# BraveGroup/DCD

Hardware: AMD Instinct MI355X
Metric: images/sec DGDE train step (bs=8, 384x1280) (higher is better)
Workload: dtype f32; 1 GPU; DGDE train bs=8 fp32 on 1xMI355X, synthetic KITTI 384x1280 + random kpts_ann (DGDE.yaml, DLA-34+DCNv2, 6 objects/image); global_batch=8, per_gpu_batch=8, input=384x1280, parallelism=dp1, dcn_precision=f32, step_launch=eager, sync_bn=False

## Files before the change

### dcd_amd/_lib.py

```python
import ctypes
import os

_HERE = os.path.dirname(os.path.abspath(__file__))
LIB_PATH = os.path.join(_HERE, "libdcd_hip.so")
_LIB = None

c_void_p, c_int, c_float, c_size_t, c_int64, c_double = (ctypes.c_void_p, ctypes.c_int, ctypes.c_float,
                                                         ctypes.c_size_t, ctypes.c_int64, ctypes.c_double)


class LossRowsArgs(ctypes.Structure):
    _INTS = ("B", "M", "C", "K", "NP", "num_classes", "ch_box2d", "ch_offset", "ch_corner", "ch_corner_unc", "ch_dims",
             "ch_ori_cls", "ch_ori_off", "ch_depth", "ch_depth_unc", "ch_kpts2d", "ch_kpts3d", "trunc_log")
    _FLOATS = ("depth_lo", "depth_hi", "unc_lo", "unc_hi", "depth_weight")
    _POINTERS = ("pois", "reg_mask", "trunc_mask", "find_pcl", "ori_mask", "cls_ids", "centers", "pad_size", "bboxes",
                 "locations", "rotys", "offset_3D", "dimensions", "orientations", "keypoints", "kp_depth_mask", "kpts2d",
                 "kpts3d", "calib_P", "calib", "dim_mean", "kps_pred", "kps_tgt", "kps3d_pred", "kps3d_tgt", "rot", "P_rows",
                 "kmask", "pair_depth", "pair_mask", "cols", "corners_pred", "corners_tgt", "iou3d", "sums", "grad_sums",
                 "grad_pois", "grad_pair", "grad_kps", "grad_kps3d")
    _fields_ = ([(n, c_int) for n in _INTS] + [(n, c_float) for n in _FLOATS] + [("dim_weight", c_float * 3)]
                + [("down_ratio", c_float), ("kd_eps", c_float)] + [(n, c_void_p) for n in _POINTERS])

HEADS_MAX = 16

# ... 48 lines not shown
    "dcd_nms_hm": (c_int, [c_void_p, c_void_p, c_int, c_int, c_int, c_int, c_void_p]),
    "dcd_heatmap_topk": (c_int, [c_void_p, c_void_p] + [c_int] * 6 + [c_void_p] * 5 + [c_void_p, c_size_t]),
    "dcd_heatmap_topk_workspace_bytes": (c_size_t, [c_int] * 5),
    "dcd_poi_gather": (c_int, [c_void_p, c_void_p, c_void_p] + [c_int] * 5 + [c_void_p]),
    "dcd_poi_scatter_add": (c_int, [c_void_p, c_void_p, c_void_p] + [c_int] * 5 + [c_void_p]),
    "dcd_patch_scatter_add": (c_int, [c_void_p, c_void_p, c_void_p, c_int, c_int, c_int64, c_int, c_int, c_void_p]),
    "dcd_iou3d": (c_int, [c_void_p, c_void_p, c_void_p, c_int, c_void_p]),
    "dcd_conv3x3_workspace_bytes": (c_size_t, [c_int] * 5),
    "dcd_conv3x3": (c_int, [c_void_p] * 6 + [c_int] * 6 + [c_void_p, c_size_t]),
    "dcd_conv3x3_weights_bytes": (c_size_t, [c_int] * 3),
    "dcd_conv3x3_transform_weights": (c_int, [c_void_p, c_void_p, c_int, c_int, c_void_p, c_void_p]),
    "dcd_conv3x3_transform_weights_table": (c_int, [c_void_p, c_void_p, c_int]),
    "dcd_conv3x3_prepared": (c_int, [c_void_p] * 6 + [c_int] * 6 + [c_void_p, c_size_t]),
    "dcd_conv3x3_split_weights_bytes": (c_size_t, [c_int] * 3),
    "dcd_conv3x3_split_transform_weights": (c_int, [c_void_p, c_void_p, c_int, c_int, c_void_p, c_void_p]),
    "dcd_conv3x3_split_transform_weights_table": (c_int, [c_void_p, c_void_p, c_int]),
    "dcd_conv3x3_split_workspace_bytes": (c_size_t, [c_int] * 5),
    "dcd_conv3x3_split_prepared": (c_int, [c_void_p] * 6 + [c_int] * 7 + [c_void_p, c_size_t]),
    "dcd_conv1x1_bf16": (c_int, [c_void_p, c_void_p, c_int, c_int, c_int, c_void_p, c_void_p, c_void_p, c_int, c_int, c_int64]),
    "dcd_conv1x1_wrw_bf16_workspace_bytes": (c_size_t, [c_int, c_int, c_int, c_int64]),
    "dcd_conv1x1_wrw_bf16": (c_int, [c_void_p, c_void_p, c_void_p, c_void_p, c_int, c_int, c_int, c_int, c_int64, c_void_p, c_size_t]),
    "dcd_conv3x3_s2_f32": (c_int, [c_void_p, c_void_p, c_void_p, c_void_p, c_int, c_int, c_int, c_int, c_int]),
    "dcd_conv3x3_s2_f32_backward_data": (c_int, [c_void_p, c_void_p, c_void_p, c_void_p, c_int, c_int, c_int, c_int, c_int]),
    "dcd_conv3x3_s2_f32_wrw_workspace_bytes": (c_size_t, [c_int, c_int, c_int, c_int, c_int]),
    "dcd_conv3x3_s2_f32_wrw": (c_int, [c_void_p, c_void_p, c_void_p, c_void_p, c_int, c_int, c_int, c_int, c_int, c_void_p, c_size_t]),
    "dcd_clip_adamw_workspace_bytes": (c_size_t, [c_int, c_void_p]),
    "dcd_clip_grad_norm_scalars": (c_int, [c_void_p, c_int, c_void_p, c_void_p, c_float, c_void_p, c_size_t, c_void_p]),
    "dcd_adamw_apply": (c_int, [c_void_p, c_int] + [c_void_p] * 7 + [c_double] * 4 + [c_void_p]),
    "dcd_conv1x1_f32": (c_int, [c_void_p, c_void_p, c_int, c_int, c_int, c_void_p, c_void_p, c_void_p, c_int, c_int, c_int64]),
    "dcd_conv1x1_wrw_f32_workspace_bytes": (c_size_t, [c_int, c_int, c_int, c_int64]),
    "dcd_conv1x1_wrw_f32": (c_int, [c_void_p, c_void_p, c_void_p, c_void_p, c_int, c_int, c_int, c_int, c_int64, c_void_p, c_size_t]),
    "dcd_conv3x3_bf16_weights_bytes": (c_size_t, [c_int] * 3),
    "dcd_conv3x3_bf16_transform_weights": (c_int, [c_void_p, c_void_p, c_int, c_int, c_void_p, c_void_p]),
    "dcd_conv3x3_bf16_transform_weights_table": (c_int, [c_void_p, c_void_p, c_int]),
    "dcd_conv3x3_bf16_workspace_bytes": (c_size_t, [c_int] * 5),
    "dcd_conv3x3_bf16_prepared": (c_int, [c_void_p] * 6 + [c_int] * 6 + [c_void_p, c_size_t]),
    "dcd_conv_stem_workspace_bytes": (c_size_t, [c_int] * 3),
    "dcd_conv_stem": (c_int, [c_void_p] * 4 + [c_int] * 7 + [c_void_p, c_size_t]),
    "dcd_conv_stem_wrw_workspace_bytes": (c_size_t, [c_int] * 3),
    "dcd_conv_stem_wrw": (c_int, [c_void_p] * 4 + [c_int] * 6 + [c_void_p, c_size_t]),
    "dcd_context_norm_forward": (c_int, [c_void_p] * 4 + [c_int, c_int, c_float]),
    "dcd_context_norm_backward": (c_int, [c_void_p] * 5 + [c_int, c_int]),
    "dcd_context_norm_relu_add_forward": (c_int, [c_void_p] * 4 + [c_int, c_int, c_float]),
    "dcd_gmw_refine": (c_int, [c_void_p] * 5 + [c_int, c_void_p, c_void_p, c_int, c_int, c_int] + [c_void_p] * 3),
    "dcd_gmw_pack_records": (c_int, [c_void_p] * 4 + [c_int, c_int, c_void_p, c_int, c_int, c_int] + [c_void_p] * 9),
    "dcd_sum_tensors": (c_int, [c_void_p, c_void_p, c_int, c_void_p, c_int64]),
    "dcd_conv3x3_wrw_workspace_bytes": (c_size_t, [c_int] * 5),
    "dcd_conv3x3_wrw": (c_int, [c_void_p] * 4 + [c_int] * 6 + [c_void_p, c_size_t]),
    "dcd_upsample_dw_forward": (c_int, [c_void_p] * 4 + [c_int] * 5),
    "dcd_upsample_dw_forward_add": (c_int, [c_void_p] * 5 + [c_int] * 5),
    "dcd_maxpool2x2_forward": (c_int, [c_void_p, c_void_p, c_void_p, c_int64, c_int, c_int]),
    "dcd_maxpool2x2_backward": (c_int, [c_void_p, c_void_p, c_void_p, c_void_p, c_int64, c_int, c_int]),
    "dcd_upsample_dw_backward": (c_int, [c_void_p] * 6 + [c_int] * 5),
    "dcd_bn_workspace_bytes": (c_size_t, [c_int]),
    "dcd_bn_stats": (c_int, [c_void_p, c_void_p, c_int, c_int, c_int64, c_void_p, c_void_p, c_size_t]),
    "dcd_channel_sums": (c_int, [c_void_p, c_void_p, c_int, c_int, c_int64, c_void_p, c_void_p, c_size_t]),
    "dcd_bn_train_apply": (c_int, [c_void_p] * 6 + [c_double] + [c_void_p] * 3 + [c_float, c_float, c_int] + [c_void_p] * 3
                           + [c_int, c_int, c_int64]),
    "dcd_bn_eval_apply": (c_int, [c_void_p] * 7 + [c_float, c_int, c_void_p, c_int, c_int, c_int64]),
    "dcd_bn_backward_stats": (c_int, [c_void_p] * 5 + [c_int, c_int, c_int64, c_void_p, c_void_p, c_size_t]),
    "dcd_trunk_row_sums": (c_int, [c_void_p, c_void_p, c_void_p, c_int, c_int, c_void_p]),
    "dcd_trunk_finalize_forward": (c_int, [c_void_p, c_void_p, c_void_p, c_void_p, c_double, c_double, c_int, c_void_p, c_void_p, c_void_p]),
    "dcd_trunk_finalize_backward": (c_int, [c_void_p, c_void_p, c_void_p, c_void_p, c_void_p, c_double, c_int, c_void_p, c_void_p, c_void_p]),
    "dcd_trunk_grad_wg": (c_int, [c_void_p, c_void_p, c_void_p, c_int, c_int, c_void_p]),
    "dcd_bn_backward_relu_from_x": (c_int, [c_void_p] * 10 + [c_int, c_int, c_int64, c_void_p, c_size_t]),
    "dcd_bn_backward_stats_params_relu_from_x": (c_int, [c_void_p] * 7 + [c_int, c_int, c_int64, c_void_p, c_void_p, c_void_p, c_void_p, c_size_t]),
    "dcd_bn_backward_apply_relu_from_x": (c_int, [c_void_p] * 8 + [c_double, c_void_p, c_int, c_int, c_int64]),
    "dcd_bn_backward_stats_params": (c_int, [c_void_p] * 6 + [c_int, c_int, c_int64, c_void_p, c_void_p, c_void_p, c_void_p, c_size_t]),
    "dcd_bn_backward_apply": (c_int, [c_void_p] * 8 + [c_double] + [c_void_p] * 4 + [c_int, c_int, c_int64]),
    "dcd_bn_at_forward": (c_int, [c_void_p] * 6 + [c_double] + [c_void_p] * 3 + [c_float, c_float, c_int] + [c_void_p] * 4
                          + [c_int, c_int, c_int64, c_int] + [c_void_p, c_size_t]),
    "dcd_bn_at_backward_sums": (c_int, [c_void_p] * 7 + [c_int, c_int, c_int] + [c_void_p, c_void_p]),
    "dcd_bn_train_forward": (c_int, [c_void_p] * 8 + [c_float, c_float, c_int] + [c_void_p] * 3 + [c_int, c_int, c_int64]
                             + [c_void_p, c_size_t]),
    "dcd_bn_backward": (c_int, [c_void_p] * 11 + [c_int, c_int, c_int64] + [c_void_p, c_size_t]),
# ... 82 lines not shown
```

### dcd_amd/csrc/conv.hip

```cpp
#include <hip/hip_runtime.h>
#include <stdint.h>
#include <stdlib.h>

#include "../../include/dcd_hip.h"
#include "tuning_env.h"
#include "lds_limit.h"
#include "bf16_split.h"

typedef float f32x16 __attribute__((ext_vector_type(16)));
typedef float f32x4 __attribute__((ext_vector_type(4)));
typedef float f32x2 __attribute__((ext_vector_type(2)));

namespace {

constexpr int WN_CH = 8;
constexpr int WN_NT = 512;

template <int TR, int TC, int NB>
struct WinoGeom {
    static constexpr int KS = 32 * NB;
    static constexpr int U = 16 * KS * WN_CH;
    static constexpr int NTILE = TR * TC;
    static constexpr int ROWS = 4 * TR + 2;
    static constexpr int Q = (2 * TC + 8) / 4;
// ... 1398 lines not shown

static bool s2_args_ok(int B, int Cin, int H, int W, int Cout)
{
    return B > 0 && Cin > 0 && Cout > 0 && H > 0 && W > 0 && (H & 1) == 0 && (W & 7) == 0 && (Cin & 15) == 0 &&
           (int64_t)Cin * H * W < (1ll << 29) && (int64_t)Cout * (H / 2) * (W / 2) < (1ll << 29);
}

int dcd_conv3x3_s2_f32(void *stream_, const float *input, const float *weight, float *output, int B, int Cin, int H, int W, int Cout)
{
    (void)hipGetLastError();
    if (!input || !weight || !output || !s2_args_ok(B, Cin, H, W, Cout)) return DCD_ERR_BAD_ARG;
    S2Args a;
    a.x = input; a.w = weight; a.y = output; a.B = B; a.C = Cin; a.H = H; a.W = W; a.K = Cout; a.Ho = H / 2; a.Wo = W / 2;
    const int zb = (Cout + 31) / 32;
    const bool small = (int64_t)((a.Ho * a.Wo + 511) / 512) * B * zb < (int64_t)device_cus();
    if (small) hipLaunchKernelGGL(s2_conv_f32<2>, dim3((unsigned)((a.Ho * a.Wo + 255) / 256), B, zb), dim3(S2_NT), 0, (hipStream_t)stream_, a);
    else hipLaunchKernelGGL(s2_conv_f32<4>, dim3((unsigned)((a.Ho * a.Wo + 511) / 512), B, zb), dim3(S2_NT), 0, (hipStream_t)stream_, a);
    return hipGetLastError() == hipSuccess ? DCD_OK : DCD_ERR_LAUNCH;
}

int dcd_conv3x3_s2_f32_backward_data(void *stream_, const float *grad_output, const float *weight, float *grad_input, int B, int Cin, int H,
                                     int W, int Cout)
{
    (void)hipGetLastError();
    if (!grad_output || !weight || !grad_input || !s2_args_ok(B, Cin, H, W, Cout) || (Cout & 15)) return DCD_ERR_BAD_ARG;
    S2Args a;
    a.x = grad_output; a.w = weight; a.y = grad_input; a.B = B; a.C = Cin; a.H = H; a.W = W; a.K = Cout; a.Ho = H / 2; a.Wo = W / 2;
    const int zb = (Cin + 31) / 32;
    const bool small = (int64_t)((a.Ho * a.Wo + 511) / 512) * B * 2 * zb < (int64_t)device_cus();
    if (small) hipLaunchKernelGGL(s2_dgrad_f32<2>, dim3((unsigned)((a.Ho * a.Wo + 255) / 256), B, 2 * zb), dim3(S2_NT), 0, (hipStream_t)stream_, a);
    else hipLaunchKernelGGL(s2_dgrad_f32<4>, dim3((unsigned)((a.Ho * a.Wo + 511) / 512), B, 2 * zb), dim3(S2_NT), 0, (hipStream_t)stream_, a);
    return hipGetLastError() == hipSuccess ? DCD_OK : DCD_ERR_LAUNCH;
}

static int s2_wrw_splits(int B, int Cin, int H, int W, int Cout)
{
    const int nblk = ((Cout + 31) / 32) * ((Cin + 31) / 32);
    const int64_t groups = (int64_t)B * (H / 2) * (W / 2) / 8;
    int64_t S = (8 * (int64_t)device_cus() + nblk - 1) / nblk;
    if (S > groups / 8) S = groups / 8;
    if (S < 1) S = 1;
    return (int)S;
}

size_t dcd_conv3x3_s2_f32_wrw_workspace_bytes(int B, int Cin, int H, int W, int Cout)
{
    if (!s2_args_ok(B, Cin, H, W, Cout)) return 0;
    return (size_t)s2_wrw_splits(B, Cin, H, W, Cout) * 9 * Cout * Cin * sizeof(float);
}

// ... 93 lines not shown
```

### dcd_amd/csrc/conv_s2_f32.inc

```

constexpr int S2_NT = 256;

struct S2Args {
    const float *x, *w;
    float *y;
    int B, C, H, W, K, Ho, Wo;
};

template <int NPX> struct S2WinT { float v[3][2 * NPX + 1]; };
typedef S2WinT<4> S2Win;

template <int NPX>
__device__ __forceinline__ void s2_gather(const __amdgpu_buffer_rsrc_t rs, const int (&off_l)[3], const int (&off_v)[3], int soff, S2WinT<NPX> &w)
{
#pragma unroll
    for (int a = 0; a < 3; ++a) {
        w.v[a][0] = __builtin_bit_cast(float, __builtin_amdgcn_raw_buffer_load_b32(rs, off_l[a], soff, 0));
        const f32x4 p = __builtin_bit_cast(f32x4, __builtin_amdgcn_raw_buffer_load_b128(rs, off_v[a], soff, 0));
        w.v[a][1] = p.x; w.v[a][2] = p.y; w.v[a][3] = p.z; w.v[a][4] = p.w;
        if constexpr (NPX == 4) {
            const f32x4 q = __builtin_bit_cast(f32x4, __builtin_amdgcn_raw_buffer_load_b128(rs, off_v[a] + 16, soff, 0));
            w.v[a][5] = q.x; w.v[a][6] = q.y; w.v[a][7] = q.z; w.v[a][8] = q.w;
        }
    }
}

template <int NPX>
__global__ __launch_bounds__(S2_NT, 2) void s2_conv_f32(S2Args a)
{
// ... 129 lines not shown
        }
        __syncthreads();
#pragma unroll
        for (int j = 0; j < 8; ++j) {
            const int kn = ck * 8 + j + DEP;
            if (kn < nk) gather(((kn >> 3) * 16 + (kn & 7)) * HWo * 4, win[(j + DEP) % NBUF]);
            const Win &w = win[j % NBUF];
#pragma unroll
            for (int ia = 0; ia < NR; ++ia) {
                const int ta = PY ? (ia == 0 ? 0 : 2) : 1, r = PY ? (ia == 0 ? 1 : 0) : 0;
#pragma unroll
                for (int tb = 0; tb < 3; ++tb) {
                    const int px = tb == 1 ? 0 : 1, dm = tb == 0 ? 1 : 0;
                    const float A = wl[((ta * 3 + tb) * 2 + (j >> 2)) * 64 + lane][j & 3];
#pragma unroll
                    for (int t = 0; t < NPX; ++t)
                        acc[px][t] = __builtin_amdgcn_mfma_f32_32x32x2f32(A, w.g[r][t + dm], acc[px][t], 0, 0, 0);
                }
            }
        }
    }
    if (!pv) return;
    float *o_b = a.y + (size_t)b * a.C * HW + (size_t)(2 * i + PY) * a.W + 2 * j0;
#pragma unroll
    for (int r = 0; r < 16; ++r) {
        const int c = z * 32 + (r & 3) + 8 * (r >> 2) + 4 * kg;
        if (c < a.C) {
            *reinterpret_cast<f32x4 *>(o_b + (size_t)c * HW) = f32x4{acc[0][0][r], acc[1][0][r], acc[0][1][r], acc[1][1][r]};
            if constexpr (NPX == 4)
                *reinterpret_cast<f32x4 *>(o_b + (size_t)c * HW + 4) = f32x4{acc[0][2][r], acc[1][2][r], acc[0][3][r], acc[1][3][r]};
        }
    }
}

template <int NPX>
__global__ __launch_bounds__(S2_NT, 2) void s2_dgrad_f32(S2Args a)
{
    __shared__ __attribute__((aligned(16))) f32x4 wl[9 * 2 * 64];
    if (blockIdx.z & 1) s2_dgrad_body<1, NPX>(a, wl, blockIdx.z >> 1);
    else s2_dgrad_body<0, NPX>(a, wl, blockIdx.z >> 1);
}

struct S2WrwArgs {
    const float *x, *gy;
    float *part;
    int B, C, H, W, K, Ho, Wo, S, ncb;
// ... 92 lines not shown
```

### dcd_amd/csrc/upsample.hip

```cpp
#include <hip/hip_runtime.h>
#include <stdlib.h>

#include <cstdint>
#include <stdint.h>

#include "../../include/dcd_hip.h"
#include "tuning_env.h"
#include "zero_fill.h"

namespace {

template <int F>
__global__ __launch_bounds__(256) void up_dw_fwd(const float *__restrict__ x, const float *__restrict__ w, float *__restrict__ y,
                                                 int C, int H, int W, const float *__restrict__ skip)
{
    constexpr int K = 2 * F, P = F / 2;
    __shared__ float ws[K * K];
    const int plane = blockIdx.y, c = plane % C;
    for (int i = threadIdx.x; i < K * K; i += 256) ws[i] = w[(size_t)c * K * K + i];
    __syncthreads();
    const int Ho = H * F, Wo = W * F;
    const float *xp = x + (size_t)plane * H * W;
    float *yp = y + (size_t)plane * Ho * Wo;
    const int o0 = (blockIdx.x * 256 + threadIdx.x) * 4;
// ... 169 lines not shown
    if (c > m || c != c) { m = c; k = 2; }
    if (d > m || d != d) { m = d; k = 3; }
    return k;
}

__global__ __launch_bounds__(256) void maxpool2_fwd(const float *__restrict__ x, float *__restrict__ y, int64_t planes, int H, int W)
{
    const int Ho = H / 2, Wq = W / 4;
    const int64_t n = planes * Ho * Wq;
    for (int64_t i = (int64_t)blockIdx.x * 256 + threadIdx.x; i < n; i += (int64_t)gridDim.x * 256) {
        const int q = (int)(i % Wq);
        const int64_t r = i / Wq;
        const int oy = (int)(r % Ho);
        const int64_t pl = r / Ho;
        const float *p = x + (pl * H + 2 * oy) * W + 4 * q;
        const float4 t = *reinterpret_cast<const float4 *>(p), b = *reinterpret_cast<const float4 *>(p + W);
        float m0, m1;
        argmax4(t.x, t.y, b.x, b.y, m0);
        argmax4(t.z, t.w, b.z, b.w, m1);
        *reinterpret_cast<float2 *>(y + (pl * Ho + oy) * (W / 2) + 2 * q) = make_float2(m0, m1);
    }
}

__global__ __launch_bounds__(256) void maxpool2_bwd(const float *__restrict__ x, const float *__restrict__ gy, float *__restrict__ gx,
                                                    int64_t planes, int H, int W)
{
    const int Ho = H / 2, Wq = W / 4;
    const int64_t n = planes * Ho * Wq;
    for (int64_t i = (int64_t)blockIdx.x * 256 + threadIdx.x; i < n; i += (int64_t)gridDim.x * 256) {
        const int q = (int)(i % Wq);
        const int64_t r = i / Wq;
        const int oy = (int)(r % Ho);
        const int64_t pl = r / Ho;
        const size_t o = (size_t)(pl * H + 2 * oy) * W + 4 * q;
        const float4 t = *reinterpret_cast<const float4 *>(x + o), b = *reinterpret_cast<const float4 *>(x + o + W);
        const float2 g = *reinterpret_cast<const float2 *>(gy + (pl * Ho + oy) * (W / 2) + 2 * q);
        float m;
        const int k0 = argmax4(t.x, t.y, b.x, b.y, m), k1 = argmax4(t.z, t.w, b.z, b.w, m);
        const float4 gt = make_float4(k0 == 0 ? g.x : 0.f, k0 == 1 ? g.x : 0.f, k1 == 0 ? g.y : 0.f, k1 == 1 ? g.y : 0.f);
        const float4 gb = make_float4(k0 == 2 ? g.x : 0.f, k0 == 3 ? g.x : 0.f, k1 == 2 ? g.y : 0.f, k1 == 3 ? g.y : 0.f);
        *reinterpret_cast<float4 *>(gx + o) = gt;
        *reinterpret_cast<float4 *>(gx + o + W) = gb;
    }
}

}

extern "C" {

int dcd_maxpool2x2_forward(void *stream_, const float *x, float *y, int64_t planes, int H, int W)
{
    (void)hipGetLastError();
    if (!x || !y || planes <= 0 || H < 2 || W < 4 || (H & 1) || (W & 3) || (((uintptr_t)x | (uintptr_t)y) & 15)) return DCD_ERR_BAD_ARG;
    const int64_t n = planes * (H / 2) * (W / 4);
    const unsigned grid = (unsigned)((n + 255) / 256 < 65535 * 4 ? (n + 255) / 256 : 65535 * 4);
    hipLaunchKernelGGL(maxpool2_fwd, dim3(grid), dim3(256), 0, (hipStream_t)stream_, x, y, planes, H, W);
    return hipGetLastError() == hipSuccess ? DCD_OK : DCD_ERR_LAUNCH;
}

int dcd_maxpool2x2_backward(void *stream_, const float *x, const float *grad_y, float *grad_x, int64_t planes, int H, int W)
{
    (void)hipGetLastError();
    if (!x || !grad_y || !grad_x || planes <= 0 || H < 2 || W < 4 || (H & 1) || (W & 3) ||
        (((uintptr_t)x | (uintptr_t)grad_y | (uintptr_t)grad_x) & 15))
        return DCD_ERR_BAD_ARG;
    const int64_t n = planes * (H / 2) * (W / 4);
    const unsigned grid = (unsigned)((n + 255) / 256 < 65535 * 4 ? (n + 255) / 256 : 65535 * 4);
    hipLaunchKernelGGL(maxpool2_bwd, dim3(grid), dim3(256), 0, (hipStream_t)stream_, x, grad_y, grad_x, planes, H, W);
    return hipGetLastError() == hipSuccess ? DCD_OK : DCD_ERR_LAUNCH;
}

static int upsample_forward(hipStream_t stream, const float *x, const float *weight, const float *skip, float *y, int B, int C, int H,
                            int W, int f)
{
    (void)hipGetLastError();
    if (!x || !weight || !y || B <= 0 || C <= 0 || H <= 0 || W <= 0 || (int64_t)B * C > 65535) return DCD_ERR_BAD_ARG;
    if ((f != 2 && f != 4 && f != 8) || ((W * f) & 3)) return DCD_ERR_BAD_ARG;
    const int no = H * f * W * f;
    dim3 grid((no / 4 + 255) / 256, B * C), block(256);
    static const bool old_fwd = dcd_env("DCD_UP_FWD_OLD") != nullptr;
    if (f == 2 && !old_fwd)
        hipLaunchKernelGGL(up_dw_fwd2_block, dim3((H * (W / 2) + 255) / 256, B * C), block, 0, stream, x, weight, y, C, H, W, skip);
    else if (f == 2) hipLaunchKernelGGL(up_dw_fwd<2>, grid, block, 0, stream, x, weight, y, C, H, W, skip);
    else if (f == 4) hipLaunchKernelGGL(up_dw_fwd<4>, grid, block, 0, stream, x, weight, y, C, H, W, skip);
    else hipLaunchKernelGGL(up_dw_fwd<8>, grid, block, 0, stream, x, weight, y, C, H, W, skip);
    return hipGetLastError() == hipSuccess ? DCD_OK : DCD_ERR_LAUNCH;
}

int dcd_upsample_dw_forward(void *stream_, const float *x, const float *weight, float *y, int B, int C, int H, int W, int f)
{
    return upsample_forward((hipStream_t)stream_, x, weight, nullptr, y, B, C, H, W, f);
}
// ... 35 lines not shown
```

### dcd_amd/model/backbone/dla_dcn.py

```python
import math
import os

import numpy as np
import torch
from torch import nn

from .DCNv2.dcn_v2 import DCN
from dcd_amd import ops
from dcd_amd.model.layers.norm import BatchNorm2d
from dcd_amd.model.layers.conv import Conv2d, DepthwiseUpsample, MaxPool2x2

BN_MOMENTUM = 0.1
_ROOT_SPLIT = os.environ.get("DCD_ROOT_SPLIT", "1") != "0"


def _bn(c, relu=False):
    return BatchNorm2d(c, momentum=BN_MOMENTUM, fuse_relu=relu)


def _relu_slot():
    return nn.Identity()


class BasicBlock(nn.Module):

    def __init__(self, inplanes, planes, stride=1, dilation=1):
        super().__init__()
        self.conv1 = Conv2d(inplanes, planes, 3, stride=stride, padding=dilation, bias=False, dilation=dilation)
        self.bn1 = _bn(planes, relu=True)
        self.relu = nn.ReLU(inplace=True)
        self.conv2 = Conv2d(planes, planes, 3, stride=1, padding=dilation, bias=False, dilation=dilation)
        self.bn2 = _bn(planes, relu=True)
        self.stride = stride

    def forward(self, x, residual=None):
        if residual is None or residual is x:
            y, residual = self.conv1.forward_with_skip(x)
        else:
            y = self.conv1(x)
        out = self.bn1(y)
        return self.bn2(self.conv2(out), residual)


class Root(nn.Module):

    def __init__(self, in_channels, out_channels, kernel_size, residual):
        super().__init__()
        self.conv = nn.Conv2d(in_channels, out_channels, 1, stride=1, bias=False, padding=(kernel_size - 1) // 2)
        self.bn = _bn(out_channels, relu=True)
        self.relu = nn.ReLU(inplace=True)
        self.residual = residual

    def forward(self, *x):
        c = self.conv
        if (_ROOT_SPLIT and x[0].is_cuda and x[0].dtype == torch.float32 and c.kernel_size == (1, 1) and c.stride == (1, 1)
                and c.padding == (0, 0) and c.bias is None and c.groups == 1):
            y = ops.conv1x1_of_cat(x, c.weight)
        else:
            y = c(torch.cat(x, 1))
        return self.bn(y, x[0] if self.residual else None)


class Tree(nn.Module):

# ... 3 lines not shown
        if root_dim == 0:
            root_dim = 2 * out_channels
        if level_root:
            root_dim += in_channels
        if levels == 1:
            self.tree1 = block(in_channels, out_channels, stride, dilation=dilation)
            self.tree2 = block(out_channels, out_channels, 1, dilation=dilation)
            self.root = Root(root_dim, out_channels, root_kernel_size, root_residual)
        else:
            self.tree1 = Tree(levels - 1, block, in_channels, out_channels, stride, root_dim=0,
                              root_kernel_size=root_kernel_size, dilation=dilation, root_residual=root_residual)
            self.tree2 = Tree(levels - 1, block, out_channels, out_channels, root_dim=root_dim + out_channels,
                              root_kernel_size=root_kernel_size, dilation=dilation, root_residual=root_residual)
        self.level_root = level_root
        self.root_dim = root_dim
        self.levels = levels
        self.downsample = MaxPool2x2(stride, stride=stride) if stride > 1 else None
        self.project = None
        if in_channels != out_channels:
            self.project = nn.Sequential(nn.Conv2d(in_channels, out_channels, 1, stride=1, bias=False), _bn(out_channels))
        self.dead_project = levels > 1 and self.project is not None

    def forward(self, x, residual=None, children=None):
        children = [] if children is None else children
        bottom = self.downsample(x) if self.downsample else x
        if self.project is not None and _ROOT_SPLIT and bottom.is_cuda and bottom.dtype == torch.float32:
            residual = self.project[1](ops.conv1x1_of_cat([bottom], self.project[0].weight))
        else:
            residual = self.project(bottom) if self.project else bottom
        if self.level_root:
            children.append(bottom)
        x1 = self.tree1(x, residual)
        if self.levels == 1:
            return self.root(self.tree2(x1), x1, *children)
        children.append(x1)
        return self.tree2(x1, children=children)


class DLA(nn.Module):

    def __init__(self, levels, channels, num_classes=1000, block=BasicBlock, residual_root=False):
        super().__init__()
        self.channels = channels
        self.num_classes = num_classes
        self.base_layer = nn.Sequential(Conv2d(3, channels[0], 7, stride=1, padding=3, bias=False),
                                        _bn(channels[0], relu=True), _relu_slot())
        self.level0 = self._make_conv_level(channels[0], channels[0], levels[0])
        self.level1 = self._make_conv_level(channels[0], channels[1], levels[1], stride=2)
        self.level2 = Tree(levels[2], block, channels[1], channels[2], 2, level_root=False, root_residual=residual_root)
        self.level3 = Tree(levels[3], block, channels[2], channels[3], 2, level_root=True, root_residual=residual_root)
        self.level4 = Tree(levels[4], block, channels[3], channels[4], 2, level_root=True, root_residual=residual_root)
        self.level5 = Tree(levels[5], block, channels[4], channels[5], 2, level_root=True, root_residual=residual_root)

    @staticmethod
    def _make_conv_level(inplanes, planes, convs, stride=1, dilation=1):
        mods = []
        for i in range(convs):
            mods += [Conv2d(inplanes, planes, 3, stride=stride if i == 0 else 1, padding=dilation, bias=False,
                            dilation=dilation), _bn(planes, relu=True), _relu_slot()]
            inplanes = planes
        return nn.Sequential(*mods)

    def forward(self, x):
        maps = []
        x = self.base_layer(x)
        for i in range(6):
            x = getattr(self, "level{}".format(i))(x)
            maps.append(x)
        return maps

    def load_pretrained_model(self, pretrain_path):
        weights = torch.load(pretrain_path, map_location="cpu")
        if isinstance(weights, dict) and "model" in weights:
            prefix = "backbone.bottom_up."
            weights = {k.replace(prefix, ""): v for k, v in weights["model"].items() if prefix in k}
        elif any(k.startswith("fc.") for k in weights):
            n_cls = len(weights[list(weights.keys())[-1]])
            self.fc = nn.Conv2d(self.channels[-1], n_cls, kernel_size=1, stride=1, padding=0, bias=True)
        self.load_state_dict(weights)


def dla34(pretrained=True, pretrain_path=None, **kwargs):
    model = DLA([1, 1, 1, 2, 2, 1], [16, 32, 64, 128, 256, 512], block=BasicBlock, **kwargs)
    if pretrained:
        if pretrain_path is None:
            raise RuntimeError("MODEL.PRETRAIN needs MODEL.PRETRAIN_PATH: this environment has no network to fetch "
                               "the ImageNet DLA-34 weights the reference downloads (dla_dcn.py:61-62)")
        model.load_pretrained_model(pretrain_path)
    return model

# ... 93 lines not shown
```

### dcd_amd/model/layers/conv.py

```python
import os

import torch
from torch import nn

from dcd_amd import ops

_ENABLED = os.environ.get("DCD_CONV_WINOGRAD", "1") != "0"
_SKIP = os.environ.get("DCD_CONV_SKIP_NODE", "1") != "0"
_STEM = os.environ.get("DCD_CONV_STEM", "1") != "0"


ROUTES = ("conv3x3", "conv3x3_with_skip", "conv3x3_stock_forward", "conv3x3_stride2_native", "conv3x3_stride2", "conv_stem",
          "conv2d_bias", "stock")


def conv2d_route(module, x, skip=False):
    if not _ENABLED or module.groups != 1 or module.padding_mode != "zeros":
        return "stock"
    w, bias = module.weight, module.bias
    if bias is None and module.kernel_size == (3, 3) and module.padding == (1, 1) and module.dilation == (1, 1):
        if module.stride == (1, 1):
            if ops.conv3x3_supported(x, w):
                return "conv3x3_with_skip" if skip and _SKIP and torch.is_grad_enabled() and x.requires_grad else "conv3x3"
            if torch.is_grad_enabled() and w.requires_grad and ops.conv3x3_wrw_only_supported(x, w):
# ... 10 lines not shown
                and (w.shape[1] == 16 or not x.requires_grad)):
            return "conv_stem"
    elif (x.is_cuda and x.dtype == torch.float32 and torch.is_grad_enabled() and bias.requires_grad
            and (x.shape[0] * x.shape[2] * x.shape[3] >= 1 << 16
                 or ops.conv3x3_bias_supported(x, w, module.stride, module.padding, module.dilation))):
        return "conv2d_bias"
    return "stock"


class Conv2d(nn.Conv2d):
    def forward(self, x):
        return self._run(conv2d_route(self, x), x)

    def _run(self, route, x):
        if route == "stock":
            ops.stock_conv_in_capture(self, x)
            return super().forward(x)
        if route == "conv2d_bias":
            return ops.conv2d_bias(x, self.weight, self.bias, self.stride, self.padding, self.dilation)
        return getattr(ops, route)(x, self.weight)

    def forward_with_skip(self, x):
        route = conv2d_route(self, x, skip=True)
        return self._run(route, x) if route == "conv3x3_with_skip" else (self._run(route, x), x)


class DepthwiseUpsample(nn.ConvTranspose2d):

    def forward_add(self, x, skip):
        f = self.stride[0]
        if self._hip_ok(x, None) and skip.is_cuda and skip.dtype == torch.float32:
            return ops.upsample_dw(x, self.weight, f, skip)
        return self.forward(x) + skip

    def _hip_ok(self, x, output_size):
        f = self.stride[0]
        return (_ENABLED and output_size is None and x.is_cuda and x.dtype == torch.float32 and self.bias is None
                and self.groups == self.in_channels == self.out_channels and self.stride == (f, f) and f in (2, 4, 8)
                and self.kernel_size == (2 * f, 2 * f) and self.padding == (f // 2, f // 2) and self.output_padding == (0, 0)
                and self.dilation == (1, 1) and (x.shape[3] * f) % 4 == 0 and x.shape[0] * x.shape[1] <= 65535)

    def forward(self, x, output_size=None):
        if self._hip_ok(x, output_size):
            return ops.upsample_dw(x, self.weight, self.stride[0])
        return super().forward(x, output_size)


class MaxPool2x2(nn.MaxPool2d):

    def forward(self, x):
        def two(v):
            return v == 2 or v == (2, 2)
        if (_ENABLED and x.is_cuda and x.dtype == torch.float32 and x.dim() == 4 and two(self.kernel_size) and two(self.stride)
                and self.padding in (0, (0, 0)) and self.dilation in (1, (1, 1)) and not self.ceil_mode and not self.return_indices
                and x.shape[2] % 2 == 0 and x.shape[3] % 4 == 0):
            return ops.maxpool2x2(x)
        return super().forward(x)
```

### dcd_amd/ops.py

```python
import os

import torch

from . import _lib
from .structures.params_3d import _typed


def _f32c(t):
    if t.dtype != torch.float32:
        t = t.float()
    return t.contiguous()


class _PairsDepth(torch.autograd.Function):
    @staticmethod
    def forward(ctx, kps, kps3d, rot_y, P, kmask, topk, zmin, zmax, normalized, sub_b3):
        _lib.require_cuda(kps, kps3d, rot_y, P)
        L = _lib.lib()
        kps, kps3d, P = _f32c(kps), _f32c(kps3d), _f32c(P)
        rot = _f32c(rot_y).reshape(-1)
        N, K = kps.shape[0], kps.shape[1]
        npairs = K * (K - 1) // 2
        M = topk if topk else npairs
        dev = kps.device
# ... 608 lines not shown
    ws = torch.empty(max(int(nbytes), 16), dtype=torch.uint8, device=M.device)
    P = torch.empty_like(M)
    iterations = torch.empty((), dtype=torch.int32, device=M.device)
    st = L.dcd_sinkhorn(_lib.stream_of(M), M.data_ptr(), r.data_ptr(), c.data_ptr(), P.data_ptr(), b, m, n, float(lmbda),
                        float(max_distance), float(tolerance), int(max_iterations), iterations.data_ptr(), ws.data_ptr(), nbytes)
    _lib.check(st, "dcd_sinkhorn")
    return P, iterations


def iou_3d(pred_corners, target_corners):
    _lib.require_cuda(pred_corners, target_corners)
    a, b = _f32c(pred_corners.detach()), _f32c(target_corners.detach())
    N = a.shape[0]
    out = torch.empty(N, dtype=torch.float32, device=a.device)
    st = _lib.lib().dcd_iou3d(_lib.stream_of(a), a.data_ptr(), b.data_ptr(), N, out.data_ptr())
    _lib.check(st, "dcd_iou3d")
    return out


def _bn_ws(C, dev):
    return torch.empty(_lib.lib().dcd_bn_workspace_bytes(C), dtype=torch.uint8, device=dev)


_BN_MASK_FROM_X = os.environ.get("DCD_BN_MASK_FROM_X", "1") != "0"


class _BatchNormAct(torch.autograd.Function):

    @staticmethod
    def forward(ctx, x, residual, weight, bias, running_mean, running_var, num_batches_tracked, momentum, eps, relu, group):
        _lib.require_cuda(x, residual, weight, bias)
        L = _lib.lib()
        x = _f32c(x)
        residual = None if residual is None else _f32c(residual)
        B, C = x.shape[0], x.shape[1]
        HW = x.numel() // (B * C)
        dev, st = x.device, _lib.stream_of(x)
        ws = _bn_ws(C, dev)
        count = float(B * HW)
        y = torch.empty_like(x)
        save_mean = torch.empty(C, dtype=torch.float32, device=dev)
        save_invstd = torch.empty(C, dtype=torch.float32, device=dev)
        if group is None:
            _lib.check(L.dcd_bn_train_forward(st, x.data_ptr(), _lib.ptr(residual), _lib.ptr(weight), _lib.ptr(bias),
                                              _lib.ptr(running_mean), _lib.ptr(running_var), _lib.ptr(num_batches_tracked),
                                              float(momentum), float(eps), int(bool(relu)), y.data_ptr(), save_mean.data_ptr(),
# ... 518 lines not shown
    B, C, H, W = x.shape
    K = weight.shape[0]
    return (H % 4 == 0 and W % 8 == 0 and W >= 16 and C % 16 == 0 and K % 16 == 0 and B * (H // 2) * (W // 2) >= _S2_NATIVE_MIN_PIXELS
            and B * max(C * H * W, K * (H // 2) * (W // 2)) < (1 << 29))


class _Conv3x3S2Native(torch.autograd.Function):

    @staticmethod
    def forward(ctx, x, weight):
        _lib.require_cuda(x, weight)
        x, weight = _f32c(x), _f32c(weight)
        B, C, H, W = x.shape
        K = weight.shape[0]
        y = torch.empty((B, K, H // 2, W // 2), dtype=torch.float32, device=x.device)
        _lib.check(_lib.lib().dcd_conv3x3_s2_f32(_lib.stream_of(x), x.data_ptr(), weight.data_ptr(), y.data_ptr(), B, C, H, W, K),
                   "dcd_conv3x3_s2_f32")
        ctx.save_for_backward(x, weight)
        return y

    @staticmethod
    @torch.autograd.function.once_differentiable
    def backward(ctx, gy):
        x, weight = ctx.saved_tensors
        gy = _f32c(gy)
        L = _lib.lib()
        B, C, H, W = x.shape
        K = weight.shape[0]
        st = _lib.stream_of(x)
        gx = gw = None
        if ctx.needs_input_grad[0]:
            gx = torch.empty_like(x)
            _lib.check(L.dcd_conv3x3_s2_f32_backward_data(st, gy.data_ptr(), weight.data_ptr(), gx.data_ptr(), B, C, H, W, K),
                       "dcd_conv3x3_s2_f32_backward_data")
        if ctx.needs_input_grad[1]:
            gw = torch.empty_like(weight)
            n = L.dcd_conv3x3_s2_f32_wrw_workspace_bytes(B, C, H, W, K)
            ws = torch.empty(max(n, 16), dtype=torch.uint8, device=x.device)
            _lib.check(L.dcd_conv3x3_s2_f32_wrw(st, x.data_ptr(), gy.data_ptr(), gw.data_ptr(), B, C, H, W, K, ws.data_ptr(), n),
                       "dcd_conv3x3_s2_f32_wrw")
        return gx, gw


def conv3x3_stride2_native(x, weight):
    return _Conv3x3S2Native.apply(x, weight)


def conv3x3_wrw_only_supported(x, weight):
    return (_WRW_ENABLED and _device_f32_kxk(x, weight) and weight.shape[0] >= 64
            and _winograd_map(x.shape[2], x.shape[3], weight.shape[1], 24 * 80) and x.shape[2] * x.shape[3] < _CONV_MIN_MAP)


class _Conv3x3StockFwd(torch.autograd.Function):

    @staticmethod
    def forward(ctx, x, weight):
        ctx.save_for_backward(x, weight)
        ctx.prec = _conv_prec(x)
        return torch.nn.functional.conv2d(x, weight, None, 1, 1)

    @staticmethod
    @torch.autograd.function.once_differentiable
    def backward(ctx, gy):
        x, weight = ctx.saved_tensors
        gy = _f32c(gy)
        gx = gw = None
        if ctx.needs_input_grad[0]:
            gx = torch.ops.aten.convolution_backward(gy, x, weight, None, [1, 1], [1, 1], [1, 1], False, [0, 0], 1,
# ... 292 lines not shown
        B, C, H, W = x.shape
        gx, gw = torch.empty_like(x), torch.empty_like(weight)
        st = _lib.lib().dcd_upsample_dw_backward(_lib.stream_of(x), x.data_ptr(), weight.data_ptr(), gy.data_ptr(), gx.data_ptr(),
                                                 gw.data_ptr(), B, C, H, W, ctx.f)
        _lib.check(st, "dcd_upsample_dw_backward")
        return gx, gw, None, (gy if ctx.has_skip else None)


class _MaxPool2x2(torch.autograd.Function):
    @staticmethod
    def forward(ctx, x):
        _lib.require_cuda(x)
        x = _f32c(x)
        B, C, H, W = x.shape
        y = torch.empty((B, C, H // 2, W // 2), dtype=torch.float32, device=x.device)
        st = _lib.lib().dcd_maxpool2x2_forward(_lib.stream_of(x), x.data_ptr(), y.data_ptr(), B * C, H, W)
        _lib.check(st, "dcd_maxpool2x2_forward")
        ctx.save_for_backward(x)
        return y

    @staticmethod
    @torch.autograd.function.once_differentiable
    def backward(ctx, gy):
        (x,) = ctx.saved_tensors
        gy = _f32c(gy)
        gx = torch.empty_like(x)
        B, C, H, W = x.shape
        st = _lib.lib().dcd_maxpool2x2_backward(_lib.stream_of(x), x.data_ptr(), gy.data_ptr(), gx.data_ptr(), B * C, H, W)
        _lib.check(st, "dcd_maxpool2x2_backward")
        return gx


def maxpool2x2(x):
    return _MaxPool2x2.apply(x)


def upsample_dw(x, weight, f, skip=None):
    return _UpsampleDW.apply(x, weight, f, skip)


class _BatchNormActAt(torch.autograd.Function):

    @staticmethod
    def forward(ctx, x, pos, weight, bias, running_mean, running_var, num_batches_tracked, momentum, eps, relu, group):
        _lib.require_cuda(x, pos, weight, bias)
        L = _lib.lib()
        x = _f32c(x)
        pos = pos.contiguous().long()
        B, C = x.shape[0], x.shape[1]
        HW = x.numel() // (B * C)
        N = pos.shape[1]
        dev, st = x.device, _lib.stream_of(x)
        ws = _bn_ws(C, dev)
        count = float(B * HW)
        stats = None
        if group is not None:
            import torch.distributed as dist
# ... 376 lines not shown
```

### include/dcd_hip.h

```cpp
#ifndef DCD_HIP_H
#define DCD_HIP_H

#include <stddef.h>
#include <stdint.h>

#ifdef __cplusplus
extern "C" {
#endif

#define DCD_OK 0
#define DCD_ERR_BAD_ARG 1
#define DCD_ERR_WORKSPACE 2
#define DCD_ERR_LAUNCH 3

const char *dcd_version(void);


#define DCD_PREC_F32 0
#define DCD_PREC_BF16X3 1
#define DCD_PREC_BF16 2

size_t dcd_dcn_v2_workspace_bytes(int B, int Cin, int H, int W, int Cout, int kh, int kw, int sh, int sw,
                                  int ph, int pw, int dh, int dw, int dg);

// ... 201 lines not shown
size_t dcd_conv3x3_bf16_weights_bytes(int Cin, int Cout, int backward_data);
int dcd_conv3x3_bf16_transform_weights(void *stream, const float *weight, int Cin, int Cout, void *forward_out, void *backward_out);
int dcd_conv3x3_bf16_transform_weights_table(void *stream, const long long *table, int entries);
size_t dcd_conv3x3_bf16_workspace_bytes(int B, int Cin, int H, int W, int Cout);
int dcd_conv3x3_bf16_prepared(void *stream, const float *input, const void *transformed, const float *bias, const float *residual,
                              float *output, int B, int Cin, int H, int W, int Cout, int backward_data, void *workspace,
                              size_t workspace_bytes);

int dcd_conv1x1_bf16(void *stream, const float *weight, int ldw, int transposed, int n_inputs, const float *const *inputs,
                     const int *channels, float *output, int B, int M, long long HW);
size_t dcd_conv1x1_wrw_bf16_workspace_bytes(int B, int O, int C, long long HW);
int dcd_conv1x1_wrw_bf16(void *stream, const float *grad_output, const float *input, float *grad_weight, int ldw, int B, int O, int C,
                         long long HW, void *workspace, size_t workspace_bytes);

int dcd_conv1x1_f32(void *stream, const float *weight, int ldw, int transposed, int n_inputs, const float *const *inputs,
                    const int *channels, float *output, int B, int M, long long HW);
size_t dcd_conv1x1_wrw_f32_workspace_bytes(int B, int O, int C, long long HW);
int dcd_conv1x1_wrw_f32(void *stream, const float *grad_output, const float *input, float *grad_weight, int ldw, int B, int O, int C,
                        long long HW, void *workspace, size_t workspace_bytes);

int dcd_conv3x3_s2_f32(void *stream, const float *input, const float *weight, float *output, int B, int Cin, int H, int W, int Cout);
int dcd_conv3x3_s2_f32_backward_data(void *stream, const float *grad_output, const float *weight, float *grad_input, int B, int Cin, int H,
                                     int W, int Cout);
size_t dcd_conv3x3_s2_f32_wrw_workspace_bytes(int B, int Cin, int H, int W, int Cout);
int dcd_conv3x3_s2_f32_wrw(void *stream, const float *input, const float *grad_output, float *grad_weight, int B, int Cin, int H, int W,
                           int Cout, void *workspace, size_t workspace_bytes);

size_t dcd_conv3x3_wrw_workspace_bytes(int B, int Cin, int H, int W, int Cout);
int dcd_conv3x3_wrw(void *stream, const float *input, const float *grad_output, float *grad_weight, int B, int Cin, int H, int W,
                    int Cout, int precision, void *workspace, size_t workspace_bytes);

size_t dcd_conv_stem_workspace_bytes(int Cin, int Cout, int ksize);
int dcd_conv_stem(void *stream, const float *input, const float *weight, float *output, int B, int Cin, int H, int W, int Cout,
                  int ksize, int backward_data, void *workspace, size_t workspace_bytes);
size_t dcd_conv_stem_wrw_workspace_bytes(int Cin, int Cout, int ksize);
int dcd_conv_stem_wrw(void *stream, const float *input, const float *grad_output, float *grad_weight, int B, int Cin, int H, int W,
                      int Cout, int ksize, void *workspace, size_t workspace_bytes);

int dcd_upsample_dw_forward(void *stream, const float *x, const float *weight, float *y, int B, int C, int H, int W, int f);
int dcd_upsample_dw_forward_add(void *stream, const float *x, const float *weight, const float *skip, float *y, int B, int C, int H,
                                int W, int f);

int dcd_maxpool2x2_forward(void *stream, const float *x, float *y, int64_t planes, int H, int W);
int dcd_maxpool2x2_backward(void *stream, const float *x, const float *grad_y, float *grad_x, int64_t planes, int H, int W);
int dcd_upsample_dw_backward(void *stream, const float *x, const float *weight, const float *grad_y, float *grad_x,
                             float *grad_weight, int B, int C, int H, int W, int f);

int dcd_encode_targets(void *stream, const double *objs, const double *kpts3d, const double *P, const int32_t *img_size,
                       const int32_t *n_obj, int B, int M, int n_extra, int in_w, int in_h, int down_ratio, double filter_trunc,
                       double filter_size, double edge_heatmap_ratio, int num_bin, int n_classes, void *const *outputs,
                       int n_outputs);

int dcd_preprocess_images(void *stream, const uint8_t *src, int64_t src_bytes, const int64_t *images, const float *table, int B,
                          int in_h, int in_w, int to_bgr, float *out);

#define DCD_EVAL_MATCH_SCORES 0
#define DCD_EVAL_MATCH_COUNTS 1
#define DCD_EVAL_MAX_THRESHOLDS 41
typedef struct {
    int mode, n_img, n_comb, n_rows, G, D, n_dc, max_dt, T, n_slots;
    int64_t P;
    const int32_t *gt_off, *dt_off, *dc_off;
    const int64_t *pair_off;
    const double *overlaps;
    const int8_t *ign_gt, *ign_dt;
    const double *dt_score, *gt_alpha, *dt_alpha, *dt_box2d, *dc_box;
    const int32_t *comb;
// ... 96 lines not shown
```

Before: 220.5 images/s.

## Fuse skip-gradient accumulation into stride-2 conv and maxpool backward kernels

When a tensor feeds both a downsampling op (stride-2 conv or 2x2 maxpool) and a skip path, such as a DLA level output that is also saved as a feature map, the two gradients were previously summed by autograd in a separate elementwise add. New autograd functions return the input as a second output, and their backward kernels read the skip gradient and add it while writing grad_input. This removes one full-size read/write pass and an allocation per join, at the cost of restructuring the DLA Tree and level forward to route through these with_skip variants, gated by the DCD_GRAD_JOIN flag.

Result: slower. 216.5 images/s (-1.8%).

```diff
diff --git a/dcd_amd/_lib.py b/dcd_amd/_lib.py
--- a/dcd_amd/_lib.py
+++ b/dcd_amd/_lib.py
@@ -94,6 +94,7 @@
     "dcd_conv1x1_wrw_bf16": (c_int, [c_void_p, c_void_p, c_void_p, c_void_p, c_int, c_int, c_int, c_int, c_int64, c_void_p, c_size_t]),
     "dcd_conv3x3_s2_f32": (c_int, [c_void_p, c_void_p, c_void_p, c_void_p, c_int, c_int, c_int, c_int, c_int]),
     "dcd_conv3x3_s2_f32_backward_data": (c_int, [c_void_p, c_void_p, c_void_p, c_void_p, c_int, c_int, c_int, c_int, c_int]),
+    "dcd_conv3x3_s2_f32_backward_data_add": (c_int, [c_void_p, c_void_p, c_void_p, c_void_p, c_void_p, c_int, c_int, c_int, c_int, c_int]),
     "dcd_conv3x3_s2_f32_wrw_workspace_bytes": (c_size_t, [c_int, c_int, c_int, c_int, c_int]),
     "dcd_conv3x3_s2_f32_wrw": (c_int, [c_void_p, c_void_p, c_void_p, c_void_p, c_int, c_int, c_int, c_int, c_int, c_void_p, c_size_t]),
     "dcd_clip_adamw_workspace_bytes": (c_size_t, [c_int, c_void_p]),
@@ -123,6 +124,7 @@
     "dcd_upsample_dw_forward_add": (c_int, [c_void_p] * 5 + [c_int] * 5),
     "dcd_maxpool2x2_forward": (c_int, [c_void_p, c_void_p, c_void_p, c_int64, c_int, c_int]),
     "dcd_maxpool2x2_backward": (c_int, [c_void_p, c_void_p, c_void_p, c_void_p, c_int64, c_int, c_int]),
+    "dcd_maxpool2x2_backward_add": (c_int, [c_void_p, c_void_p, c_void_p, c_void_p, c_void_p, c_int64, c_int, c_int]),
     "dcd_upsample_dw_backward": (c_int, [c_void_p] * 6 + [c_int] * 5),
     "dcd_bn_workspace_bytes": (c_size_t, [c_int]),
     "dcd_bn_stats": (c_int, [c_void_p, c_void_p, c_int, c_int, c_int64, c_void_p, c_void_p, c_size_t]),
diff --git a/dcd_amd/csrc/conv.hip b/dcd_amd/csrc/conv.hip
--- a/dcd_amd/csrc/conv.hip
+++ b/dcd_amd/csrc/conv.hip
@@ -1444,10 +1444,18 @@
 int dcd_conv3x3_s2_f32_backward_data(void *stream_, const float *grad_output, const float *weight, float *grad_input, int B, int Cin, int H,
                                      int W, int Cout)
 {
-    (void)hipGetLastError();
-    if (!grad_output || !weight || !grad_input || !s2_args_ok(B, Cin, H, W, Cout) || (Cout & 15)) return DCD_ERR_BAD_ARG;
+    return dcd_conv3x3_s2_f32_backward_data_add(stream_, grad_output, weight, nullptr, grad_input, B, Cin, H, W, Cout);
+}
+
+int dcd_conv3x3_s2_f32_backward_data_add(void *stream_, const float *grad_output, const float *weight, const float *addend, float *grad_input,
+                                         int B, int Cin, int H, int W, int Cout)
+{
+    (void)hipGetLastError();
+    if (!grad_output || !weight || !grad_input || !s2_args_ok(B, Cin, H, W, Cout) || (Cout & 15) || ((uintptr_t)addend & 15))
+        return DCD_ERR_BAD_ARG;
     S2Args a;
     a.x = grad_output; a.w = weight; a.y = grad_input; a.B = B; a.C = Cin; a.H = H; a.W = W; a.K = Cout; a.Ho = H / 2; a.Wo = W / 2;
+    a.add = addend;
     const int zb = (Cin + 31) / 32;
     const bool small = (int64_t)((a.Ho * a.Wo + 511) / 512) * B * 2 * zb < (int64_t)device_cus();
     if (small) hipLaunchKernelGGL(s2_dgrad_f32<2>, dim3((unsigned)((a.Ho * a.Wo + 255) / 256), B, 2 * zb), dim3(S2_NT), 0, (hipStream_t)stream_, a);
diff --git a/dcd_amd/csrc/conv_s2_f32.inc b/dcd_amd/csrc/conv_s2_f32.inc
--- a/dcd_amd/csrc/conv_s2_f32.inc
+++ b/dcd_amd/csrc/conv_s2_f32.inc
@@ -5,6 +5,7 @@
     const float *x, *w;
     float *y;
     int B, C, H, W, K, Ho, Wo;
+    const float *add = nullptr;
 };
 
 template <int NPX> struct S2WinT { float v[3][2 * NPX + 1]; };
@@ -180,6 +181,30 @@
     }
     if (!pv) return;
     float *o_b = a.y + (size_t)b * a.C * HW + (size_t)(2 * i + PY) * a.W + 2 * j0;
+    if (a.add) {
+        const float *d_b = a.add + (size_t)b * a.C * HW + (size_t)(2 * i + PY) * a.W + 2 * j0;
+#pragma unroll
+        for (int r0 = 0; r0 < 16; r0 += 4) {
+            f32x4 q[4][NPX / 2];
+#pragma unroll
+            for (int u = 0; u < 4; ++u) {
+                const int c = z * 32 + ((r0 + u) & 3) + 8 * ((r0 + u) >> 2) + 4 * kg;
+#pragma unroll
+                for (int h = 0; h < NPX / 2; ++h)
+                    q[u][h] = c < a.C ? *reinterpret_cast<const f32x4 *>(d_b + (size_t)c * HW + 4 * h) : f32x4{0.f, 0.f, 0.f, 0.f};
+            }
+#pragma unroll
+            for (int u = 0; u < 4; ++u) {
+                const int r = r0 + u, c = z * 32 + (r & 3) + 8 * (r >> 2) + 4 * kg;
+                if (c >= a.C) continue;
+#pragma unroll
+                for (int h = 0; h < NPX / 2; ++h)
+                    *reinterpret_cast<f32x4 *>(o_b + (size_t)c * HW + 4 * h) =
+                        f32x4{acc[0][2 * h][r], acc[1][2 * h][r], acc[0][2 * h + 1][r], acc[1][2 * h + 1][r]} + q[u][h];
+            }
+        }
+        return;
+    }
 #pragma unroll
     for (int r = 0; r < 16; ++r) {
         const int c = z * 32 + (r & 3) + 8 * (r >> 2) + 4 * kg;
diff --git a/dcd_amd/csrc/upsample.hip b/dcd_amd/csrc/upsample.hip
--- a/dcd_amd/csrc/upsample.hip
+++ b/dcd_amd/csrc/upsample.hip
@@ -215,7 +215,8 @@
     }
 }
 
-__global__ __launch_bounds__(256) void maxpool2_bwd(const float *__restrict__ x, const float *__restrict__ gy, float *__restrict__ gx,
+template <bool ADD>
+__global__ __launch_bounds__(256) void maxpool2_bwd(const float *__restrict__ x, const float *__restrict__ gy, float *gx, const float *addend,
                                                     int64_t planes, int H, int W)
 {
     const int Ho = H / 2, Wq = W / 4;
@@ -232,8 +233,14 @@
         const int k0 = argmax4(t.x, t.y, b.x, b.y, m), k1 = argmax4(t.z, t.w, b.z, b.w, m);
         const float4 gt = make_float4(k0 == 0 ? g.x : 0.f, k0 == 1 ? g.x : 0.f, k1 == 0 ? g.y : 0.f, k1 == 1 ? g.y : 0.f);
         const float4 gb = make_float4(k0 == 2 ? g.x : 0.f, k0 == 3 ? g.x : 0.f, k1 == 2 ? g.y : 0.f, k1 == 3 ? g.y : 0.f);
-        *reinterpret_cast<float4 *>(gx + o) = gt;
-        *reinterpret_cast<float4 *>(gx + o + W) = gb;
+        if constexpr (ADD) {
+            const float4 at = *reinterpret_cast<const float4 *>(addend + o), ab = *reinterpret_cast<const float4 *>(addend + o + W);
+            *reinterpret_cast<float4 *>(gx + o) = make_float4(gt.x + at.x, gt.y + at.y, gt.z + at.z, gt.w + at.w);
+            *reinterpret_cast<float4 *>(gx + o + W) = make_float4(gb.x + ab.x, gb.y + ab.y, gb.z + ab.z, gb.w + ab.w);
+        } else {
+            *reinterpret_cast<float4 *>(gx + o) = gt;
+            *reinterpret_cast<float4 *>(gx + o + W) = gb;
+        }
     }
 }
 
@@ -251,16 +258,23 @@
     return hipGetLastError() == hipSuccess ? DCD_OK : DCD_ERR_LAUNCH;
 }
 
-int dcd_maxpool2x2_backward(void *stream_, const float *x, const float *grad_y, float *grad_x, int64_t planes, int H, int W)
+int dcd_maxpool2x2_backward_add(void *stream_, const float *x, const float *grad_y, const float *addend, float *grad_x, int64_t planes,
+                                int H, int W)
 {
     (void)hipGetLastError();
     if (!x || !grad_y || !grad_x || planes <= 0 || H < 2 || W < 4 || (H & 1) || (W & 3) ||
-        (((uintptr_t)x | (uintptr_t)grad_y | (uintptr_t)grad_x) & 15))
+        (((uintptr_t)x | (uintptr_t)grad_y | (uintptr_t)grad_x | (uintptr_t)addend) & 15))
         return DCD_ERR_BAD_ARG;
     const int64_t n = planes * (H / 2) * (W / 4);
     const unsigned grid = (unsigned)((n + 255) / 256 < 65535 * 4 ? (n + 255) / 256 : 65535 * 4);
-    hipLaunchKernelGGL(maxpool2_bwd, dim3(grid), dim3(256), 0, (hipStream_t)stream_, x, grad_y, grad_x, planes, H, W);
+    if (addend) hipLaunchKernelGGL(maxpool2_bwd<true>, dim3(grid), dim3(256), 0, (hipStream_t)stream_, x, grad_y, grad_x, addend, planes, H, W);
+    else hipLaunchKernelGGL(maxpool2_bwd<false>, dim3(grid), dim3(256), 0, (hipStream_t)stream_, x, grad_y, grad_x, addend, planes, H, W);
     return hipGetLastError() == hipSuccess ? DCD_OK : DCD_ERR_LAUNCH;
+}
+
+int dcd_maxpool2x2_backward(void *stream_, const float *x, const float *grad_y, float *grad_x, int64_t planes, int H, int W)
+{
+    return dcd_maxpool2x2_backward_add(stream_, x, grad_y, nullptr, grad_x, planes, H, W);
 }
 
 static int upsample_forward(hipStream_t stream, const float *x, const float *weight, const float *skip, float *y, int B, int C, int H,
diff --git a/dcd_amd/model/backbone/dla_dcn.py b/dcd_amd/model/backbone/dla_dcn.py
--- a/dcd_amd/model/backbone/dla_dcn.py
+++ b/dcd_amd/model/backbone/dla_dcn.py
@@ -40,6 +40,12 @@
             y = self.conv1(x)
         out = self.bn1(y)
         return self.bn2(self.conv2(out), residual)
+
+    def forward_with_tail(self, x, residual=None):
+        if residual is None or residual is x:
+            return self.forward(x, residual), x
+        y, tail = self.conv1.forward_with_skip(x)
+        return self.bn2(self.conv2(self.bn1(y)), residual), tail
 
 
 class Root(nn.Module):
@@ -89,6 +95,8 @@
         self.dead_project = levels > 1 and self.project is not None
 
     def forward(self, x, residual=None, children=None):
+        if ops._GRAD_JOIN:
+            return self.forward_with_tail(x, residual, children)[0]
         children = [] if children is None else children
         bottom = self.downsample(x) if self.downsample else x
         if self.project is not None and _ROOT_SPLIT and bottom.is_cuda and bottom.dtype == torch.float32:
@@ -102,6 +110,24 @@
             return self.root(self.tree2(x1), x1, *children)
         children.append(x1)
         return self.tree2(x1, children=children)
+
+    def forward_with_tail(self, x, residual=None, children=None):
+        children = [] if children is None else children
+        if self.downsample:
+            bottom, x = self.downsample.forward_with_skip(x)
+        else:
+            bottom = x
+        if self.project is not None and _ROOT_SPLIT and bottom.is_cuda and bottom.dtype == torch.float32:
+            residual = self.project[1](ops.conv1x1_of_cat([bottom], self.project[0].weight))
+        else:
+            residual = self.project(bottom) if self.project else bottom
+        if self.level_root:
+            children.append(bottom)
+        x1, tail = self.tree1.forward_with_tail(x, residual)
+        if self.levels == 1:
+            return self.root(self.tree2(x1), x1, *children), tail
+        children.append(x1)
+        return self.tree2(x1, children=children), tail
 
 
 class DLA(nn.Module):
@@ -132,7 +158,11 @@
         maps = []
         x = self.base_layer(x)
         for i in range(6):
-            x = getattr(self, "level{}".format(i))(x)
+            level = getattr(self, "level{}".format(i))
+            if ops._GRAD_JOIN and isinstance(level, Tree) and maps:
+                x, maps[-1] = level.forward_with_tail(x)
+            else:
+                x = level(x)
             maps.append(x)
         return maps
 
diff --git a/dcd_amd/model/layers/conv.py b/dcd_amd/model/layers/conv.py
--- a/dcd_amd/model/layers/conv.py
+++ b/dcd_amd/model/layers/conv.py
@@ -56,7 +56,11 @@
 
     def forward_with_skip(self, x):
         route = conv2d_route(self, x, skip=True)
-        return self._run(route, x) if route == "conv3x3_with_skip" else (self._run(route, x), x)
+        if route == "conv3x3_with_skip":
+            return self._run(route, x)
+        if route == "conv3x3_stride2_native" and ops._GRAD_JOIN and torch.is_grad_enabled() and x.requires_grad:
+            return ops.conv3x3_stride2_native_with_skip(x, self.weight)
+        return self._run(route, x), x
 
 
 class DepthwiseUpsample(nn.ConvTranspose2d):
@@ -82,11 +86,19 @@
 
 class MaxPool2x2(nn.MaxPool2d):
 
-    def forward(self, x):
+    def _hip_ok(self, x):
         def two(v):
             return v == 2 or v == (2, 2)
-        if (_ENABLED and x.is_cuda and x.dtype == torch.float32 and x.dim() == 4 and two(self.kernel_size) and two(self.stride)
+        return (_ENABLED and x.is_cuda and x.dtype == torch.float32 and x.dim() == 4 and two(self.kernel_size) and two(self.stride)
                 and self.padding in (0, (0, 0)) and self.dilation in (1, (1, 1)) and not self.ceil_mode and not self.return_indices
-                and x.shape[2] % 2 == 0 and x.shape[3] % 4 == 0):
+                and x.shape[2] % 2 == 0 and x.shape[3] % 4 == 0)
+
+    def forward(self, x):
+        if self._hip_ok(x):
             return ops.maxpool2x2(x)
         return super().forward(x)
+
+    def forward_with_skip(self, x):
+        if self._hip_ok(x) and ops._GRAD_JOIN and torch.is_grad_enabled() and x.requires_grad:
+            return ops.maxpool2x2_with_skip(x)
+        return self.forward(x), x
diff --git a/dcd_amd/ops.py b/dcd_amd/ops.py
--- a/dcd_amd/ops.py
+++ b/dcd_amd/ops.py
@@ -654,6 +654,7 @@
     return torch.empty(_lib.lib().dcd_bn_workspace_bytes(C), dtype=torch.uint8, device=dev)
 
 
+_GRAD_JOIN = os.environ.get("DCD_GRAD_JOIN", "1") != "0"
 _BN_MASK_FROM_X = os.environ.get("DCD_BN_MASK_FROM_X", "1") != "0"
 
 
@@ -1218,6 +1219,10 @@
     @staticmethod
     @torch.autograd.function.once_differentiable
     def backward(ctx, gy):
+        return _Conv3x3S2Native.run_backward(ctx, gy)
+
+    @staticmethod
+    def run_backward(ctx, gy, gskip=None):
         x, weight = ctx.saved_tensors
         gy = _f32c(gy)
         L = _lib.lib()
@@ -1227,8 +1232,9 @@
         gx = gw = None
         if ctx.needs_input_grad[0]:
             gx = torch.empty_like(x)
-            _lib.check(L.dcd_conv3x3_s2_f32_backward_data(st, gy.data_ptr(), weight.data_ptr(), gx.data_ptr(), B, C, H, W, K),
-                       "dcd_conv3x3_s2_f32_backward_data")
+            gskip = None if gskip is None else _f32c(gskip)
+            _lib.check(L.dcd_conv3x3_s2_f32_backward_data_add(st, gy.data_ptr(), weight.data_ptr(), _lib.ptr(gskip), gx.data_ptr(),
+                                                              B, C, H, W, K), "dcd_conv3x3_s2_f32_backward_data")
         if ctx.needs_input_grad[1]:
             gw = torch.empty_like(weight)
             n = L.dcd_conv3x3_s2_f32_wrw_workspace_bytes(B, C, H, W, K)
@@ -1238,8 +1244,26 @@
         return gx, gw
 
 
+class _Conv3x3S2NativeSkip(torch.autograd.Function):
+
+    @staticmethod
+    def forward(ctx, x, weight):
+        return _Conv3x3S2Native.forward(ctx, x, weight), x.view_as(x)
+
+    @staticmethod
+    @torch.autograd.function.once_differentiable
+    def backward(ctx, gy, gskip):
+        if gy is None:
+            return gskip, None
+        return _Conv3x3S2Native.run_backward(ctx, gy, gskip if ctx.needs_input_grad[0] else None)
+
+
 def conv3x3_stride2_native(x, weight):
     return _Conv3x3S2Native.apply(x, weight)
+
+
+def conv3x3_stride2_native_with_skip(x, weight):
+    return _Conv3x3S2NativeSkip.apply(x, weight)
 
 
 def conv3x3_wrw_only_supported(x, weight):
@@ -1578,17 +1602,41 @@
     @staticmethod
     @torch.autograd.function.once_differentiable
     def backward(ctx, gy):
+        return _MaxPool2x2.run_backward(ctx, gy)
+
+    @staticmethod
+    def run_backward(ctx, gy, gskip=None):
         (x,) = ctx.saved_tensors
         gy = _f32c(gy)
         gx = torch.empty_like(x)
         B, C, H, W = x.shape
-        st = _lib.lib().dcd_maxpool2x2_backward(_lib.stream_of(x), x.data_ptr(), gy.data_ptr(), gx.data_ptr(), B * C, H, W)
+        gskip = None if gskip is None else _f32c(gskip)
+        st = _lib.lib().dcd_maxpool2x2_backward_add(_lib.stream_of(x), x.data_ptr(), gy.data_ptr(), _lib.ptr(gskip), gx.data_ptr(),
+                                                    B * C, H, W)
         _lib.check(st, "dcd_maxpool2x2_backward")
         return gx
 
 
+class _MaxPool2x2Skip(torch.autograd.Function):
+
+    @staticmethod
+    def forward(ctx, x):
+        return _MaxPool2x2.forward(ctx, x), x.view_as(x)
+
+    @staticmethod
+    @torch.autograd.function.once_differentiable
+    def backward(ctx, gy, gskip):
+        if gy is None:
+            return gskip
+        return _MaxPool2x2.run_backward(ctx, gy, gskip)
+
+
 def maxpool2x2(x):
     return _MaxPool2x2.apply(x)
+
+
+def maxpool2x2_with_skip(x):
+    return _MaxPool2x2Skip.apply(x)
 
 
 def upsample_dw(x, weight, f, skip=None):
diff --git a/include/dcd_hip.h b/include/dcd_hip.h
--- a/include/dcd_hip.h
+++ b/include/dcd_hip.h
@@ -247,6 +247,8 @@
 int dcd_conv3x3_s2_f32(void *stream, const float *input, const float *weight, float *output, int B, int Cin, int H, int W, int Cout);
 int dcd_conv3x3_s2_f32_backward_data(void *stream, const float *grad_output, const float *weight, float *grad_input, int B, int Cin, int H,
                                      int W, int Cout);
+int dcd_conv3x3_s2_f32_backward_data_add(void *stream, const float *grad_output, const float *weight, const float *addend,
+                                         float *grad_input, int B, int Cin, int H, int W, int Cout);
 size_t dcd_conv3x3_s2_f32_wrw_workspace_bytes(int B, int Cin, int H, int W, int Cout);
 int dcd_conv3x3_s2_f32_wrw(void *stream, const float *input, const float *grad_output, float *grad_weight, int B, int Cin, int H, int W,
                            int Cout, void *workspace, size_t workspace_bytes);
@@ -268,6 +270,8 @@
 
 int dcd_maxpool2x2_forward(void *stream, const float *x, float *y, int64_t planes, int H, int W);
 int dcd_maxpool2x2_backward(void *stream, const float *x, const float *grad_y, float *grad_x, int64_t planes, int H, int W);
+int dcd_maxpool2x2_backward_add(void *stream, const float *x, const float *grad_y, const float *addend, float *grad_x, int64_t planes,
+                                int H, int W);
 int dcd_upsample_dw_backward(void *stream, const float *x, const float *weight, const float *grad_y, float *grad_x,
                              float *grad_weight, int B, int C, int H, int W, int f);
 
```
